# CaiLiLab/MuRaL

Measured on AMD Instinct MI355X. Metric: predicted bases/s (SNV local=10/distal=1000, 4-class, predict), higher is better.
Workload: dtype f32; 1 GPU; SNV default predict, synthetic 10M positions (BASELINE.json configs[1]); local_radius=10, distal_radius=1000, n_class=4, input=2-bit packed genome resident in HBM, every site's full window, weights=weights_init, torch.manual_seed(0), parallelism=dp1, collective=none

## Files before the change

include/mural_hip_debug.h:

```cpp
#ifndef MURAL_HIP_DEBUG_H
#define MURAL_HIP_DEBUG_H
#include "mural_hip.h"

#ifdef __cplusplus
extern "C" {
#endif

int mural_debug_last_ws_layout(size_t* out_pairs, int32_t max_pairs);

int mural_debug_run_scan(int64_t* v, int64_t m, int64_t stride, int32_t threads, int64_t* total, void* stream);

int mural_debug_cl_conv32_fwd(const float* x, int64_t B, int32_t L, int32_t pre_relu, const double* acc, const float* gamma,
                              const float* beta, float* running_mean, float* running_var, float* state, const float* W,
                              const float* bias, int32_t post_relu, const float* res1, const float* res2, double* acc_out,
                              int32_t out_relu, float* y, void* stream);
int mural_debug_cl_conv32_bwd(const float* dy, const float* x, const float* W, int64_t B, int32_t L, const float* state,
                              int32_t pre_relu, float* dz, double* stat_out, float* part, int32_t* nrow, void* stream);
int mural_debug_cl_bn_stats(const float* x, int64_t rows, int32_t relu, double* acc, void* stream);
int mural_debug_first_fwd_cl(const uint8_t* sym, int64_t B, int32_t Lwin, int32_t col0, int32_t L1, int32_t pk, int32_t ps, int32_t pp,
                             const float* gamma, const float* beta, const float* W, const float* bias, float eps, float momentum,
                             float* running_mean, float* running_var, unsigned long long* counts, float* tab, float* y, void* arg,
                             double* stat, void* stream);
int mural_debug_first_bwd_cl(const float* dy, const void* arg, const uint8_t* sym, int64_t B, int32_t Lwin, int32_t col0, int32_t L1,
                             int32_t pk, int32_t ps, int32_t pp, const float* tab, const float* W, float* scratch, float* dW,
// ... 28 lines not shown
                              int32_t out_relu, float* y, float* wfrag_scratch, void* stream);
int mural_debug_cw_conv32_bwd(const float* dy, const float* x, const float* W, int64_t B, int32_t L, const float* state,
                              const float* gamma, int32_t pre_relu, float* dz, double* stat_out, float* part, int32_t* nrow,
                              float* wfrag_scratch, void* stream);

int mural_debug_conv1d(const float* in, const float* wt, const float* bias, float* out, int64_t B, int32_t Cin, int32_t Lin,
                       int32_t Cout, int32_t Lout, int32_t K, int32_t stride, int32_t up, int32_t act, const float* res1,
                       const float* res2, int32_t engine, void* stream);

int mural_debug_poison_lds(void* stream);

int mural_debug_convblock(const float* x, const float* w5, const float* b5, const float* w1, const float* b1, const float* res2,
                          float* out, int64_t B, int32_t C, int32_t L, const float* f_in, const float* f_w, const float* f_b,
                          int32_t Cf, int32_t f_up, const float* f_pw, const float* ta_w, const float* ta_b, const float* tb_w,
                          const float* tb_b, float* tail_max, int32_t form, void* stream);

int mural_debug_conv1d_set_stamps(unsigned long long* stamps);
int mural_debug_cb8_set_stamps(unsigned long long* stamps);

int mural_debug_set_stamps(void* dev_ptr);

int mural_debug_list_switches(char* buf, size_t cap);

#ifdef __cplusplus
}
#endif
#endif
```

mural_amd/_lib.py:

```python
import ctypes as C
import os

import torch

_HERE = os.path.dirname(os.path.abspath(__file__))
LIB_PATH = os.path.join(_HERE, "libmural_hip.so")

MURAL_OK, MURAL_E_INVALID, MURAL_E_RUNTIME, MURAL_E_WORKSPACE, MURAL_E_ENCODING = 0, 1, 2, 3, 4

_f32p = C.POINTER(C.c_float)


class MuralGenome(C.Structure):
    _fields_ = [("packed2", C.c_void_p), ("nmask", C.c_void_p), ("length", C.c_int64), ("amb_pos", C.c_void_p),
                ("amb_sym", C.c_void_p), ("n_amb", C.c_int64)]


class MuralBN(C.Structure):
    _fields_ = [("weight", C.c_void_p), ("bias", C.c_void_p), ("running_mean", C.c_void_p), ("running_var", C.c_void_p)]


class MuralAffine(C.Structure):
    _fields_ = [("weight", C.c_void_p), ("bias", C.c_void_p)]

# ... 315 lines not shown
    "mural_debug_first_set_stamps": (C.c_int, [VP]),
    "mural_debug_lt_set_stamps": (C.c_int, [VP]),
    "mural_debug_cw_conv32_fwd": (C.c_int, [VP, I64, I32, I32, VP, VP, VP, VP, VP, VP, VP, VP, I32, VP, VP, VP, I32, VP, VP, VP]),
    "mural_debug_cw_conv32_bwd": (C.c_int, [VP, VP, VP, I64, I32, VP, VP, I32, VP, VP, VP, VP, VP, VP]),
    "mural_debug_cl_bn_stats": (C.c_int, [VP, I64, I32, VP, VP]),
    "mural_debug_local_train_fwd": (C.c_int, [VP, VP, I32, I32, I64, VP, VP, VP, VP, VP, VP, VP, VP, VP, VP, VP, VP, C.c_float, C.c_float, VP,
                                              VP, VP, VP]),
    "mural_debug_local_train_bwd": (C.c_int, [VP, I32, I32, I64, VP, VP, VP, VP, VP, VP, VP, VP, VP, VP, VP, VP, VP, VP, VP, VP, VP, VP, VP]),
    "mural_debug_head_train_fwd": (C.c_int, [VP, I64, I32, VP, VP, VP, VP, VP, C.c_float, C.c_float, VP, VP, VP, C.c_float, C.c_uint64, VP, VP,
                                             VP, VP, I32, VP, VP]),
    "mural_debug_head_train_bwd": (C.c_int, [VP, VP, I32, I64, I32, VP, VP, VP, C.c_float, C.c_uint64, VP, VP, VP, VP, VP, VP, VP, VP, VP, VP,
                                             VP, VP]),
    "mural_debug_first_fwd_cl": (C.c_int, [VP, I64, I32, I32, I32, I32, I32, I32, VP, VP, VP, VP, C.c_float, C.c_float, VP, VP, VP, VP, VP, VP,
                                           VP, VP]),
    "mural_debug_first_bwd_cl": (C.c_int, [VP, VP, VP, I64, I32, I32, I32, I32, I32, I32, VP, VP, VP, VP, VP, VP, VP, VP, VP, VP, VP, VP, VP,
                                           VP, C.c_double, VP, VP, VP]),
    "mural_debug_conv1d": (C.c_int, [VP, VP, VP, VP, I64, I32, I32, I32, I32, I32, I32, I32, I32, VP, VP, I32, VP]),
    "mural_debug_conv1d_set_stamps": (C.c_int, [VP]),
    "mural_debug_poison_lds": (C.c_int, [VP]),
    "mural_debug_convblock": (C.c_int, [VP, VP, VP, VP, VP, VP, VP, I64, I32, I32, VP, VP, VP, I32, I32, VP, VP, VP, VP, VP, VP, I32, VP]),
    "mural_debug_cb8_set_stamps": (C.c_int, [VP]),
    "mural_debug_set_stamps": (C.c_int, [C.c_void_p]),
    "mural_debug_list_switches": (C.c_int, [C.c_char_p, C.c_size_t]),
}

_lib = None
DEBUG_LIB_PATH = os.path.join(_HERE, "libmural_hip_debug.so")


def flavor():
    return "debug" if os.environ.get("MURAL_HIP_FLAVOR", "") == "debug" else "product"


def lib():
    global _lib
    if _lib is None:
        debug = flavor() == "debug"
        path = DEBUG_LIB_PATH if debug else LIB_PATH
        if not os.path.exists(path):
            raise RuntimeError(
                f"{path} is missing: the HIP extension has not been built. "
                "Run `make -C mural_amd/csrc` (needs hipcc, --offload-arch=gfx950). There is no CPU fallback.")
        handle = C.CDLL(path)
        protos = dict(PROTOTYPES, **DEBUG_PROTOTYPES) if debug else PROTOTYPES
        for name, (res, args) in protos.items():
            fn = getattr(handle, name)
# ... 25 lines not shown
```

mural_amd/csrc/debug_hooks.hip:

```cpp
#include <cstring>
#include <string>
#include <vector>

#include "../../include/mural_hip_debug.h"
#include "common.h"
#include "conv1d.h"
#include "conv32_cl.h"
#include "conv32_jobs.h"
#include "snv.h"
#include "train_ops.h"

using namespace mural;

#define STREAM ((hipStream_t)stream)

namespace {
struct EnableDevSwitches {
  EnableDevSwitches() { mural::g_dev_switches = true; }
} g_enable_dev_switches;
}

extern "C" int mural_debug_list_switches(char* buf, size_t cap) {
  std::string text;
  int n = 0;
  for (const mural::DevSwitch* s = mural::dev_switch_table(); s->name; ++s, ++n) text += std::string(s->name) + "\t" + s->what + "\n";
  if (buf && cap) {
    std::strncpy(buf, text.c_str(), cap - 1);
    buf[cap - 1] = '\0';
  }
  return n;
}

__global__ __launch_bounds__(256) void lds_poison_kernel(float* sink) {
  extern __shared__ float lds_all[];
  for (int i = threadIdx.x; i < 160 * 256; i += 256) lds_all[i] = __builtin_nanf("");
  __syncthreads();
  if (sink && lds_all[(threadIdx.x * 97) % (160 * 256)] == 1.f) sink[0] = 1.f;
}
static int poison_lds(hipStream_t stream) {
  MURAL_HIP_CHECK(hipFuncSetAttribute(reinterpret_cast<const void*>(lds_poison_kernel), hipFuncAttributeMaxDynamicSharedMemorySize, 160 * 1024));
  hipLaunchKernelGGL(lds_poison_kernel, dim3(2048), dim3(256), 160 * 1024, stream, (float*)nullptr);
  MURAL_HIP_CHECK(hipGetLastError());
  return MURAL_OK;
}

extern "C" int mural_debug_conv1d_set_stamps(unsigned long long* stamps) {
  mural::conv1d_mfma_set_stamps(stamps);
  return MURAL_OK;
}

extern "C" int mural_debug_cb8_set_stamps(unsigned long long* stamps) {
  mural::g_cb8_stamps = stamps;
  return MURAL_OK;
// ... 239 lines not shown
```

mural_amd/csrc/encode.hip:

```cpp
#include <cstring>
#include <cstdlib>
#include "common.h"
#include "dense_symbol.h"

namespace mural {

static thread_local std::string g_err;

void set_error(const char* fmt, ...) {
  char buf[1024];
  va_list ap;
  va_start(ap, fmt);
  vsnprintf(buf, sizeof(buf), fmt, ap);
  va_end(ap);
  g_err = buf;
}

const char* last_error_cstr() { return g_err.c_str(); }

bool g_dev_switches = false;

const DevSwitch* dev_switch_table() {
  static const DevSwitch table[] = {
    {"MURAL_TOWER_DYNAMIC_UNITS", "A/B, bit-identical: SNV predict units through a global ticket counter instead of the fixed stride"},
    {"MURAL_SNV_DEFER_SHORT", "A/B, bit-identical: =0 runs the short-stage launches per chunk (what a one-chunk workspace does by itself)"},
    {"MURAL_LOCAL_REG", "A/B, bit-identical: =0 keeps the local MLP's weight fragments in LDS (snv_local_mlp_mfma)"},
    {"MURAL_INDEL_CHUNK", "A/B, same results: positions per pass of the INDEL layer program (256 .. 4096; default 2048)"},
    {"MURAL_TRAIN_CONV_CL", "A/B: the training step on the workgroup-tile conv kernels (conv32_cl.hip) instead of the wave-private ones"},
    {"MURAL_TRAIN_NO_FIRST_FOLD", "A/B: the first stage's last BatchNorm-backward apply as a pass of its own"},
    {"MURAL_TRAIN_NO_MID_FOLD", "A/B: the short stage's last apply as a pass of its own"},
    {"MURAL_TRAIN_NO_POOL_FOLD", "A/B: the applies in front of the pools as passes of their own"},
    {"MURAL_TRAIN_LOCAL_OPS", "A/B: the local branch of the training step as per-op launches"},
    {"MURAL_TRAIN_HEAD_OPS", "A/B: a tower's head of the training step as per-op launches"},
    {"MURAL_TRAIN_FIRST_SEPARATE", "A/B: symbol histograms / first-layer tables per tower"},
    {"MURAL_XCD_SWIZZLE", "A/B, bit-identical: =0 disables the XCD-aware workgroup index of the barrier-free INDEL kernels"},
    {"MURAL_CONVBLOCK_DIRECT", "A/B: 0 / 2 never / always the barrier-free ConvBlock"},
    {"MURAL_CONVBLOCK8_VALU", "A/B: the 8-channel ConvBlock entirely on the vector ALU"},
    {"MURAL_INDEL_ENC0", "A/B: =0 disables the persistent level-0 encoder launch"},
    {"MURAL_INDEL_ENC0_DOWN", "A/B: =0 keeps the stride-4 down-conv a launch of its own"},
    {"MURAL_INDEL_DEC0", "A/B: =0 disables the persistent level-0 decoder launch"},
    {"MURAL_INDEL_DEEP", "A/B: =0 runs the deep levels' blocks as two launches each"},
    {"MURAL_INDEL_DEEP_FRONT", "A/B: =0 keeps the fourth level's strided conv a launch of its own"},
    {"MURAL_INDEL_DENSE_SYMBOLS", "A/B: =0 keeps the dense INDEL entry on the three-launch route"},
    {"MURAL_WGRAD_MFMA", "A/B: =0 keeps the INDEL weight gradients on the LDS-tiled vector kernel"},
    {"MURAL_DEBUG_WS_GUARD", "validation: unused bytes behind every workspace region (tests poison and check them)"},
    {"MURAL_DEBUG_DROP_PART_ROW", "validation (fault injection): drop one partial row of a conv weight gradient"},
    {"MURAL_DEBUG_NO_SMALL_BATCH", "validation: calls of <= 256 sites through the throughput launches"},
    {"MURAL_DEBUG_NO_LONGWIN", "validation: long windows through the per-layer path"},
// ... 240 lines not shown
```

mural_amd/csrc/snv.h:

```cpp
#pragma once
#include "common.h"

namespace mural {

constexpr int SNV_C = 32;
constexpr int SNV_K = 3;
constexpr int SNV_NLAYER = 10;
constexpr int SNV_KSTEPS = 24;
constexpr int SNV_WFRAG = 2 * SNV_KSTEPS * 64;
constexpr int SNV_LUT = 125 * SNV_C;
constexpr int SNV_TAPS = 3 * N_SYM * SNV_C;
constexpr int SNV_LUTBLK = SNV_LUT + SNV_TAPS + SNV_C;
constexpr int SNV_LUT4 = 256 * SNV_C;
constexpr int SNV_MAXCLASS = 16;
constexpr int SNV_CHUNK = 131072;
constexpr int SNV_NB2MAX = 9;
constexpr int SNV_THREADS = 256;
constexpr int SNV_WAVES = SNV_THREADS / 64;
constexpr int SNV_MID_HALF = 100;

enum { L_RB1A_C1 = 0, L_RB1A_C2, L_RB1B_C1, L_RB1B_C2, L_CONV2, L_RB2A_C1, L_RB2A_C2, L_RB2B_C1, L_RB2B_C2, L_CONV3 };
enum { EX_RB1_ENTRY = 0, EX_BN_MID = 1, EX_BN_OUT = 2, EX_FC_BN = 3, EX_COUNT = 4 };

struct TowerGeom {
// ... 172 lines not shown
  float* blob;
  size_t blob_floats;
  size_t lds_bytes;
  mural::Stage1Args s1;
  size_t s1_lds_bytes;
  bool s1_pair;
  bool loc_fused;
  mural::LocalMfmaDims loc_d;
  size_t loc_lds;
  bool longwin;
  bool front_only;
  bool front_mid;
  int lw_nA, lw_LA, lw_LB, lw_SB, lw_nj;
  mural::SnvFwdArgs args_lwA, args_lwB;
  size_t lds_lwA, lds_lwB;
  int64_t chunk;
};

namespace mural {
bool stage1_small_batch(int64_t n);
int launch_snv_stage1(const Stage1Args& a, bool packed, size_t lds_bytes, hipStream_t stream);
int launch_snv_local(const LocalDev& L, const int64_t* cat, int64_t n, float* out, hipStream_t stream);
int launch_snv_towers(const MuralSnvModel* m, const SnvFwdArgs& a, size_t lds_bytes, hipStream_t stream);
int profile_begin();
int profile_end(double* total_ms, int64_t* launches);
size_t plan_wave_geometry(SnvFwdArgs& a, int Lwin, int Pw, int n_class, int tower, int phase);
int launch_snv_tower_wave(const SnvFwdArgs& a, size_t lds_bytes, hipStream_t stream);
int launch_snv_tower_wave_jobs(const SnvFwdArgs* jobs, const size_t* lds_bytes, int n, hipStream_t stream);
extern unsigned long long* g_tower_stamps;
}
```

mural_amd/csrc/snv_model.hip:

```cpp
#include <algorithm>
#include <cmath>
#include <cstdio>
#include <cstdlib>
#include <cstring>
#include <vector>

#include "snv.h"
#include "snv_local_mfma.h"

namespace mural {

namespace {

const double kSymVec[15][4] = {
    {1, 0, 0, 0}, {0, 1, 0, 0}, {0, 0, 1, 0}, {0, 0, 0, 1}, {.25, .25, .25, .25},
    {.5, 0, .5, 0}, {0, .5, 0, .5}, {.5, .5, 0, 0}, {0, .5, .5, 0}, {.5, 0, 0, .5}, {0, 0, .5, .5},
    {0, 1. / 3, 1. / 3, 1. / 3}, {1. / 3, 0, 1. / 3, 1. / 3}, {1. / 3, 1. / 3, 0, 1. / 3}, {1. / 3, 1. / 3, 1. / 3, 0}};

struct Blob {
  std::vector<float> host;
  size_t alloc(size_t n) {
    size_t off = (host.size() + 63) & ~size_t(63);
    host.resize(off + n, 0.f);
    return off;
// ... 341 lines not shown
          if (need && need <= kLdsTwoPerCu) { Pq = cand; m->lds_split[q] = need; }
        }
        if (!Pq) return false;
        if (phase == 2) {
          for (int cand = Pq; cand >= Pq - 2 && cand >= 1; --cand) {
            SnvFwdArgs tmp;
            const size_t need = plan_geometry(tmp, sh.distal_len, cand, sh.n_class, towers, phase);
            if (need && tmp.geom[q & 1].nb[1] % 4 == 0) { Pq = cand; m->lds_split[q] = need; break; }
          }
        }
        plan_geometry(m->args_split[q], sh.distal_len, Pq, sh.n_class, towers, phase);
        for (int cand = 31; cand >= 1; --cand) {
          SnvFwdArgs tmp;
          std::memset(&tmp, 0, sizeof(tmp));
          const size_t need = plan_wave_geometry(tmp, sh.distal_len, cand, sh.n_class, q & 1, phase);
          if (need && need <= kLdsTwoPerCu) {
            m->args_split[q] = tmp;
            m->lds_split[q] = need;
            break;
          }
        }
        return true;
      };
      m->chunk = SNV_CHUNK;
      m->longwin = false;
      if (!dev_env("MURAL_DEBUG_NO_LONGWIN")) {
        SnvFwdArgs probe;
        std::memset(&probe, 0, sizeof(probe));
        fill_tower_lengths(probe, sh.distal_len);
        const int L2 = probe.geom[0].L[0], nj = 19, LA = 7 * nj + 8;
        if (L2 > LA && probe.geom[0].pk[1] == 7 && probe.geom[0].ps[1] == 7 && probe.geom[0].pp[1] == 3) {
          int nA = 0;
          while (7 * nj * nA + LA <= L2) ++nA;
          const int SB = 7 * ((L2 - 142 + 6) / 7), LB = L2 - SB;
          bool ok = nA >= 1 && LB >= 127 && LB <= 142 && SB <= 7 * nj * nA && SB >= 0;
          if (ok) {
            std::memset(&m->args_lwA, 0, sizeof(SnvFwdArgs));
            std::memset(&m->args_lwB, 0, sizeof(SnvFwdArgs));
            m->lds_lwA = plan_wave_geometry(m->args_lwA, 15 * (LA - 1) + 1, 1, sh.n_class, 0, 1);
            m->lds_lwB = plan_wave_geometry(m->args_lwB, 15 * (LB - 1) + 1, 1, sh.n_class, 0, 1);
            ok = m->lds_lwA && m->lds_lwA <= kLdsTwoPerCu && m->lds_lwB && m->lds_lwB <= kLdsTwoPerCu &&
                 m->args_lwA.geom[0].L[0] == LA && m->args_lwB.geom[0].L[0] == LB;
          }
          bool part_ok[4] = {ok, false, false, false};
          for (int q = 1; q < 4 && ok; ++q) part_ok[q] = plan_part(q);
          const bool short_ok = ok && part_ok[1] && part_ok[2] && part_ok[3];
          if (ok) {
// ... 127 lines not shown
extern "C" int mural_snv_tap_layout(const MuralSnvModel* m, int32_t* o) {
  MURAL_REQUIRE(m && o, "NULL argument");
  std::memset(o, 0, 16 * sizeof(int32_t));
  o[0] = m->args.P;
  o[1] = m->args.nbuf;
  for (int i = 0; i < 3; ++i) { o[2 + i] = m->args.geom[0].L[i]; o[5 + i] = m->args.geom[1].L[i]; }
  o[8] = 13;
  o[9] = (int32_t)m->lds_bytes;
  o[10] = m->front_only ? 1 : 0;
  o[11] = (int32_t)m->chunk;
  o[12] = m->front_mid ? 1 : 0;
  return MURAL_OK;
}

extern "C" const char* mural_snv_kernel_name(void) { return "snv_tower_wave"; }

extern "C" int mural_profile_begin(void) { return mural::profile_begin(); }
extern "C" int mural_profile_end(double* total_ms, int64_t* launches) { return mural::profile_end(total_ms, launches); }

namespace mural { unsigned long long* g_tower_stamps = nullptr; }

constexpr int64_t SNV_SMALL_BATCH = 256;

static int run_towers(const MuralSnvModel* m, Stage1Args s1, SnvFwdArgs a, bool packed, int64_t n, const Workspace& w,
                      float* out, float* taps, const int32_t* status, hipStream_t stream, bool one_chunk = false, float* front_out = nullptr) {
  const int nc = m->shape.n_class;
  const bool small = taps == nullptr && n <= SNV_SMALL_BATCH && m->lds_small > 0 && !dev_env("MURAL_DEBUG_NO_SMALL_BATCH");
  const bool defer = m->split && taps == nullptr && !small && !m->longwin && super_chunk_sites(m) > m->chunk && n > m->chunk && !one_chunk;
  const int64_t super = defer ? super_chunk_sites(m) : m->chunk;
  const size_t s3l_site = (size_t)std::max(m->args.geom[0].L[1], 1) * SNV_C, s3m_site = (size_t)std::max(m->args.geom[1].L[1], 1) * SNV_C;
  for (int64_t sc0 = 0; sc0 < n; sc0 += super) {
  const int64_t sn = std::min<int64_t>(super, n - sc0);
  for (int64_t c0 = sc0; c0 < sc0 + sn; c0 += m->chunk) {
    const int64_t cn = std::min<int64_t>(m->chunk, sc0 + sn - c0);
    const int64_t rel = defer ? c0 - sc0 : 0;
    Stage1Args s = s1;
    s.n = cn;
    s.x0 = w.x0;
    s.zero = small ? reinterpret_cast<int*>(w.s3[1]) : nullptr;
    if (packed) { s.pos = s1.pos + c0; s.strand = s1.strand + c0; }
    else s.codes = s1.codes + c0 * m->shape.distal_len;
    if (int rc = launch_snv_stage1(s, packed, s.loc_on ? std::max(m->s1_lds_bytes, m->loc_lds) : m->s1_lds_bytes, stream)) return rc;
    const bool split = m->split && taps == nullptr && !small;
    if (split && dev_int("MURAL_TOWER_DYNAMIC_UNITS", 0) != 0)
      MURAL_HIP_CHECK(hipMemsetAsync(w.counters, 0, 64, stream));
    bool lw_mid_done = false;
    for (int part = 0; part < (split ? (defer ? 2 : 4) : 1); ++part) {
      if (part == 1 && lw_mid_done) continue;
      if (m->longwin && part == 0) {
        const int LpA = m->args_lwA.geom[0].L[1], LpB = m->args_lwB.geom[0].L[1], L3 = m->args.geom[0].L[1], nj = m->lw_nj;
        const int x0_cols = m->args.x0_cols;
        auto grid_of = [](int64_t items) { return dim3((unsigned)std::min<int64_t>((items + 255) / 256, 65536)); };
        SnvFwdArgs lw_jobs[3];
        size_t lw_lds[3];
        const bool lw_merge = m->args_lwA.wave && m->args_lwB.wave && m->args_split[1].wave && (!front_out || m->front_mid);
        for (int kind = 0; kind < 2; ++kind) {
          SnvFwdArgs t = kind == 0 ? m->args_lwA : m->args_lwB;
          t.n = kind == 0 ? cn * m->lw_nA : cn;
          t.x0 = w.x0;
          t.x0_cols = x0_cols;
          t.seg_n = kind == 0 ? m->lw_nA : 1;
          t.seg_step = kind == 0 ? 7 * nj : 0;
          t.seg_col0 = kind == 0 ? 0 : m->lw_SB;
          t.s3[0] = kind == 0 ? w.vs3A : w.vs3B;
          t.s3[1] = w.s3[1];
          t.xlogit = w.xlogit;
          t.local_logits = w.local_logits + c0 * nc;
          t.out = out ? out + c0 * nc : nullptr;
          t.taps = nullptr;
          t.stamps = nullptr;
// ... 16 lines not shown
          t.local_logits = w.local_logits + c0 * nc;
          t.out = out ? out + c0 * nc : nullptr;
          t.taps = nullptr;
          t.tap_stride = a.nbuf;
          t.stamps = nullptr;
          t.status = status;
          t.unit_counter = nullptr;
          lw_jobs[2] = t;
          lw_lds[2] = m->lds_split[1];
          if (int rc = launch_snv_tower_wave_jobs(lw_jobs, lw_lds, 3, stream)) return rc;
          lw_mid_done = true;
        }
        const int jA = m->lw_nA * nj + 1;
        float* s3_dst = front_out ? front_out + (size_t)c0 * L3 * SNV_C : w.s3[0];
        hipLaunchKernelGGL(lw_scatter_kernel, grid_of(cn * jA * 8), dim3(256), 0, stream, w.vs3A, cn, m->lw_nA, LpA, nj, 0, jA, 0, L3, s3_dst);
        if (L3 > jA)
          hipLaunchKernelGGL(lw_scatter_kernel, grid_of(cn * (L3 - jA) * 8), dim3(256), 0, stream, w.vs3B, cn, 1, LpB, nj, jA, L3,
                             -(m->lw_SB / 7), L3, s3_dst);
        MURAL_HIP_CHECK(hipGetLastError());
        if (front_out && !m->front_mid) break;
        continue;
      }
      if (front_out && part > 1) break;
      SnvFwdArgs t = split ? m->args_split[part] : (small ? m->args_small : a);
      t.s3[0] = w.s3[0] + (size_t)rel * s3l_site;
      t.s3[1] = w.s3[1] + (size_t)rel * s3m_site;
      t.n = cn;
      t.x0 = w.x0;
      t.xlogit = w.xlogit + (size_t)rel * SNV_MAXCLASS;
      if (small) {
        t.par = 1;
        t.xlogit2 = w.s3[0];
        t.tile_count = reinterpret_cast<int*>(w.s3[1]);
      }
      t.local_logits = w.local_logits + c0 * nc;
      t.out = out ? out + c0 * nc : nullptr;
      t.taps = c0 == 0 ? taps : nullptr;
      t.tap_stride = a.nbuf;
      t.stamps = packed ? mural::g_tower_stamps : nullptr;
      t.status = status;
      t.unit_counter = split && t.wave ? w.counters + part : nullptr;
      size_t lds = split ? m->lds_split[part] : (small ? m->lds_small : m->lds_bytes);
      if (split && !t.wave && part >= 2 && t.P > 1) {
        const int want = (int)std::max<int64_t>(1, std::min<int64_t>(t.P, (cn + 511) / 512));
        if (want < t.P) {
          SnvFwdArgs t2 = t;
          const size_t need = plan_geometry(t2, m->shape.distal_len, want, m->shape.n_class, (part & 1) ? 2 : 1, 2);
          if (need && need <= lds) {
            t = t2;
            lds = need;
          }
        }
      }
      if (int rc = launch_snv_towers(m, t, lds, stream)) return rc;
    }
  }
  if (defer) {
    for (int part = 2; part < 4; ++part) {
      SnvFwdArgs t = m->args_split[part];
      t.s3[0] = w.s3[0];
      t.s3[1] = w.s3[1];
      t.n = sn;
      t.x0 = w.x0;
      t.xlogit = w.xlogit;
// ... 191 lines not shown
```

mural_amd/csrc/snv_tower.hip:

```cpp
#include <cstdlib>
#include <vector>

#include "snv_tower_conv.h"

namespace mural {

#define SNV_STAMP(id)                                                              \
  do {                                                                             \
    if (args.stamps != nullptr && tid == 0) {                                      \
      const unsigned long long _t = __builtin_amdgcn_s_memtime();                  \
      args.stamps[(size_t)blockIdx.x * 32 + (id)] += _t - t_prev;                  \
      t_prev = _t;                                                                 \
    }                                                                              \
  } while (0)

__device__ __forceinline__ void request_x0(const SnvFwdArgs& args, f32x4 (&xres)[SNV_NB2MAX], int64_t tile, int tw_i,
                                           int64_t n_tiles, int cgp, int n16, int chv) {
  const TowerGeom& g = args.geom[tw_i];
  const int x0c = tw_i == 0 ? 0 : args.geom[0].L[0];
  const int nbw0 = g.nb[0] > cgp ? (g.nb[0] - cgp + 1) / 2 : 0;
  const float* base = args.x0 + (size_t)x0c * 32 + chv;
#pragma unroll
  for (int i = 0; i < SNV_NB2MAX; ++i) {
    xres[i] = splat(0.f);
// ... 379 lines not shown
}

int profile_begin() {
  g_prof.on = true;
  g_prof.used = 0;
  return MURAL_OK;
}

int profile_end(double* total_ms, int64_t* launches) {
  double sum = 0.0;
  for (size_t i = 0; i + 1 < g_prof.used; i += 2) {
    MURAL_HIP_CHECK(hipEventSynchronize(g_prof.ev[i + 1]));
    float ms = 0.f;
    MURAL_HIP_CHECK(hipEventElapsedTime(&ms, g_prof.ev[i], g_prof.ev[i + 1]));
    sum += ms;
  }
  if (total_ms) *total_ms = sum;
  if (launches) *launches = (int64_t)(g_prof.used / 2);
  g_prof.on = false;
  g_prof.used = 0;
  return MURAL_OK;
}

int launch_snv_towers(const MuralSnvModel* m, const SnvFwdArgs& a, size_t lds_bytes, hipStream_t stream) {
  const int64_t n_tiles = (a.n + a.P - 1) / a.P;
  if (n_tiles == 0) return MURAL_OK;
  if (a.wave) {
    hipEvent_t w0 = nullptr, w1 = nullptr;
    if (g_prof.on) {
      while (g_prof.ev.size() < g_prof.used + 2) {
        hipEvent_t e;
        MURAL_HIP_CHECK(hipEventCreate(&e));
        g_prof.ev.push_back(e);
      }
      w0 = g_prof.ev[g_prof.used];
      w1 = g_prof.ev[g_prof.used + 1];
      g_prof.used += 2;
      MURAL_HIP_CHECK(hipEventRecord(w0, stream));
    }
    if (int rc = launch_snv_tower_wave(a, lds_bytes, stream)) return rc;
    if (w1) MURAL_HIP_CHECK(hipEventRecord(w1, stream));
    return MURAL_OK;
  }
  int grid = (int)(n_tiles < 2048 ? n_tiles : 2048);
  if (a.par) grid = (int)(2 * n_tiles);
  static DynLdsOnce big_lds;
  if (int rc = big_lds.ensure(&snv_towers_fused<0>, &snv_towers_fused<1>, &snv_towers_fused<2>, &snv_towers_fused<3>)) return rc;
  hipEvent_t e0 = nullptr, e1 = nullptr;
  if (g_prof.on) {
    while (g_prof.ev.size() < g_prof.used + 2) {
      hipEvent_t e;
      MURAL_HIP_CHECK(hipEventCreate(&e));
      g_prof.ev.push_back(e);
    }
    e0 = g_prof.ev[g_prof.used];
    e1 = g_prof.ev[g_prof.used + 1];
    g_prof.used += 2;
    MURAL_HIP_CHECK(hipEventRecord(e0, stream));
  }
  if (a.par) hipLaunchKernelGGL(snv_towers_fused<3>, dim3(grid), dim3(SNV_THREADS), lds_bytes, stream, a);
  else if (a.phase == 1) hipLaunchKernelGGL(snv_towers_fused<1>, dim3(grid), dim3(SNV_THREADS), lds_bytes, stream, a);
  else if (a.phase == 2) hipLaunchKernelGGL(snv_towers_fused<2>, dim3(grid), dim3(SNV_THREADS), lds_bytes, stream, a);
  else hipLaunchKernelGGL(snv_towers_fused<0>, dim3(grid), dim3(SNV_THREADS), lds_bytes, stream, a);
  MURAL_HIP_CHECK(hipGetLastError());
  if (e1) MURAL_HIP_CHECK(hipEventRecord(e1, stream));
  return MURAL_OK;
}

}
```

mural_amd/csrc/snv_tower_wave.hip:

```cpp
#include <cstdlib>
#include <cstring>
#include <type_traits>

#include "snv_tower_conv.h"

namespace mural {

template <int M>
using ModeTag = std::integral_constant<int, M>;
__host__ __device__ constexpr TowerGeom wave_tower_geom(int tw, int Lwin, int Pw) {
  constexpr int pools[2][3][3] = {{{15, 15, 7}, {7, 7, 3}, {3, 3, 1}}, {{3, 3, 1}, {3, 3, 1}, {3, 3, 1}}};
  TowerGeom g{};
  g.L1 = tw == 0 ? Lwin : 2 * SNV_MID_HALF + 1;
  g.col0 = tw == 0 ? 0 : Lwin / 2 - SNV_MID_HALF;
  int L = g.L1;
  for (int i = 0; i < 3; ++i) {
    g.pk[i] = pools[tw][i][0];
    g.ps[i] = pools[tw][i][1];
    g.pp[i] = pools[tw][i][2];
    L = (L + 2 * g.pp[i] - g.pk[i]) / g.ps[i] + 1;
    g.L[i] = L;
    if (L < 1) return g;
    g.Sc[i] = L + 1;
    g.NC[i] = 1 + Pw * g.Sc[i];
    g.nb[i] = (g.NC[i] + 15) / 16;
    g.dL[i] = FastDiv::make((uint32_t)L);
    g.dSc[i] = FastDiv::make((uint32_t)g.Sc[i]);
  }
  return g;
}
constexpr int SHIP_LWIN = 2001;

constexpr int MODE_GENERIC = -1;
constexpr int TW_NBW = 9;
constexpr int TW_DUMP = 128;
constexpr uint32_t TW_BLK = 2048u;

struct WaveAddr {
  uint32_t rd[6];
  uint32_t wr[2];
  uint32_t vmask;
  uint32_t dump;
};

__device__ __forceinline__ WaveAddr wave_setup(const TowerGeom& g, int st, int Pw, int n16, int kk, uint32_t dump0) {
  WaveAddr a;
  a.dump = dump0 + 16u * (uint32_t)((16 * kk + n16) & 31);
#pragma unroll
// ... 262 lines not shown
template <int PHASE, int NBA, int NBB, int TWC = -1, int PWC = 0>
__global__ __launch_bounds__(SNV_THREADS, 2) void snv_tower_wave(const SnvFwdArgs args) {
#define SNVW_BX blockIdx.x
#define SNVW_GX gridDim.x
#include "snv_tower_wave_body.inc"
}
#undef SNVW_BX
#undef SNVW_GX

struct SnvFwdJobs {
  SnvFwdArgs j[3];
  int grid[3];
};
static_assert(sizeof(SnvFwdJobs) <= 4096, "kernel arguments: 4 KB");
#define SNVW_BX bx_job
#define SNVW_GX gx_job
template <int PHASE, int NBA, int NBB, int TWC = -1, int PWC = 0>
__global__ __launch_bounds__(SNV_THREADS, 2) void snv_tower_wave_jobs(const SnvFwdJobs jobs) {
  const SnvFwdArgs& args = jobs.j[blockIdx.y];
  const unsigned gx_job = (unsigned)jobs.grid[blockIdx.y];
  const unsigned bx_job = blockIdx.x;
  if (bx_job >= gx_job) return;
#include "snv_tower_wave_body.inc"
}
#undef SNVW_BX
#undef SNVW_GX

constexpr int EW_NB = 9;
constexpr int EW_WST = 32;

__device__ __forceinline__ int64_t edge_wave_wstart(const EdgeArgs& args, int64_t row) {
  if (row >= args.n) return -1;
  const int64_t gp = args.pos[row];
  const int neg = args.strand[row] != 0;
  const int64_t t = neg ? args.glen - 1 - gp : gp;
  const int64_t w = t + args.woff - args.t0[neg];
  if (w < 0 || w + args.L1 > args.nb || args.F[neg] == nullptr) return -1;
  return w | ((int64_t)neg << 62);
}

__device__ __forceinline__ void edge_wave_request(const EdgeArgs& args, const int64_t* wst, f32x4 (&xr0)[TW_NBW], f32x4 (&xr1)[TW_NBW],
                                                  int n16_in, int kk) {
  int n16 = n16_in;
  asm volatile("" : "+v"(n16));
  const float* safe = args.F[0] != nullptr ? args.F[0] : args.F[1];
#pragma unroll
// ... 214 lines not shown
static bool tower_dynamic_units() { return dev_int("MURAL_TOWER_DYNAMIC_UNITS", 0) != 0; }

size_t edge_wave_lds_bytes() {
  return (size_t)(4 * SNV_C + 4 * 3 * SNV_C + SNV_WAVES * ((16 * EW_NB + 2) * SNV_C + EW_WST + TW_DUMP)) * 4;
}

int launch_snv_edge_wave(const EdgeArgs& e, int* unit_counter, hipStream_t stream) {
  const int64_t n_units = (e.n + EW_P - 1) / EW_P;
  const int64_t n_wg = (n_units + SNV_WAVES - 1) / SNV_WAVES;
  if (n_wg == 0) return MURAL_OK;
  const int grid = (int)(n_wg < 512 ? n_wg : 512);
  if (n_units < 4 * (int64_t)grid * SNV_WAVES || !tower_dynamic_units()) unit_counter = nullptr;
  static DynLdsOnce lds;
  if (int rc = lds.ensure(&snv_edge_wave)) return rc;
  hipLaunchKernelGGL(snv_edge_wave, dim3(grid), dim3(SNV_THREADS), edge_wave_lds_bytes(), stream, e, unit_counter);
  MURAL_HIP_CHECK(hipGetLastError());
  return MURAL_OK;
}

size_t plan_wave_geometry(SnvFwdArgs& a, int Lwin, int Pw, int n_class, int tower, int phase) {
  int maxcols = 0;
  for (int tw = 0; tw < 2; ++tw) {
    a.geom[tw] = wave_tower_geom(tw, Lwin, Pw);
    const TowerGeom& g = a.geom[tw];
    for (int i = 0; i < 3; ++i) {
      if (g.L[i] < 1) return 0;
      if (tw != tower) continue;
      if ((phase == 1 && i != 0) || (phase == 2 && i == 0)) continue;
      if (g.nb[i] > TW_NBW) return 0;
      if (phase == 1 && g.nb[i] != TW_NBW) return 0;
      maxcols = std::max(maxcols, 16 * g.nb[i] + 2);
    }
  }
  if (Pw > 31) return 0;
  if (phase == 2 && !(Lwin == SHIP_LWIN && Pw == (tower == 0 ? 6 : 5))) return 0;
  a.P = Pw;
  a.Lwin = Lwin;
  a.tw_first = tower;
  a.tw_last = tower;
  a.phase = phase;
  a.wave = 1;
  a.x0_cols = a.geom[0].L[0] + a.geom[1].L[0];
  a.nbuf = maxcols * SNV_C;
  const size_t par = (size_t)(2 * EX_COUNT * SNV_C + n_class * SNV_C + SNV_MAXCLASS + 4 + 6 * 3 * SNV_C);
  const size_t per_wave = (size_t)a.nbuf + (phase == 2 ? (size_t)Pw * SNV_C + 3 * (size_t)Pw * SNV_MAXCLASS : 0) + TW_DUMP;
  return (par + SNV_WAVES * per_wave) * 4;
// ... 10 lines not shown
    const SnvFwdArgs& a = jobs_in[i];
    MURAL_REQUIRE(a.phase == 1 && a.Lwin != SHIP_LWIN, "wave-private tower jobs: first-stage launches of the run-time-geometry instance only");
    const int64_t n_units = (a.n + a.P - 1) / a.P;
    const int64_t n_wg = (n_units + SNV_WAVES - 1) / SNV_WAVES;
    if (n_wg == 0) continue;
    jobs.j[ny] = a;
    jobs.j[ny].unit_counter = nullptr;
    wg_of[ny] = n_wg;
    lds = lds_bytes[i] > lds ? lds_bytes[i] : lds;
    ++ny;
  }
  if (ny == 0) return MURAL_OK;
  for (int i = 0; i < ny; ++i) {
    jobs.grid[i] = (int)(wg_of[i] < 512 ? wg_of[i] : 512);
    gx = jobs.grid[i] > gx ? jobs.grid[i] : gx;
  }
  static DynLdsOnce big_lds;
  if (int rc = big_lds.ensure(&snv_tower_wave_jobs<1, 9, 0>)) return rc;
  hipLaunchKernelGGL((snv_tower_wave_jobs<1, 9, 0>), dim3(gx, ny), dim3(SNV_THREADS), lds, stream, jobs);
  MURAL_HIP_CHECK(hipGetLastError());
  return MURAL_OK;
}

int launch_snv_tower_wave(const SnvFwdArgs& a_in, size_t lds_bytes, hipStream_t stream) {
  SnvFwdArgs a = a_in;
  const int64_t n_units = (a.n + a.P - 1) / a.P;
  const int64_t n_wg = (n_units + SNV_WAVES - 1) / SNV_WAVES;
  if (n_wg == 0) return MURAL_OK;
  const int resident = 512;
  const int grid = (int)(n_wg < resident ? n_wg : resident);
  if (n_units < 4 * (int64_t)grid * SNV_WAVES || !tower_dynamic_units()) a.unit_counter = nullptr;
  static DynLdsOnce big_lds;
  if (int rc = big_lds.ensure(&snv_tower_wave<1, 9, 0, 0, 1>, &snv_tower_wave<1, 9, 0, 1, 2>, &snv_tower_wave<2, 8, 4, 0, 6>,
                              &snv_tower_wave<2, 8, 3, 1, 5>, &snv_tower_wave<1, 9, 0>)) return rc;
  const int t = a.tw_first;
  const int ship_pw = a.phase == 1 ? (t == 0 ? 1 : 2) : (t == 0 ? 6 : 5);
  bool ship = a.Lwin == SHIP_LWIN && a.P == ship_pw && !(a.phase == 1 && dev_env("MURAL_DEBUG_TOWER_RUNTIME_GEOM"));
  if (ship) {
    const TowerGeom want = wave_tower_geom(t, SHIP_LWIN, ship_pw), other = wave_tower_geom(0, SHIP_LWIN, 1);
    const TowerGeom& have = a.geom[t];
    for (int i = 0; i < 3; ++i)
      ship = ship && have.L[i] == want.L[i] && have.Sc[i] == want.Sc[i] && have.NC[i] == want.NC[i] && have.nb[i] == want.nb[i] &&
             have.pk[i] == want.pk[i] && have.ps[i] == want.ps[i] && have.pp[i] == want.pp[i];
    ship = ship && a.geom[0].L[0] == other.L[0] && a.x0_cols == other.L[0] + wave_tower_geom(1, SHIP_LWIN, 1).L[0];
  }
  const dim3 gr(grid), bl(SNV_THREADS);
  if (a.phase == 1) {
    if (ship && t == 0) hipLaunchKernelGGL((snv_tower_wave<1, 9, 0, 0, 1>), gr, bl, lds_bytes, stream, a);
    else if (ship) hipLaunchKernelGGL((snv_tower_wave<1, 9, 0, 1, 2>), gr, bl, lds_bytes, stream, a);
    else hipLaunchKernelGGL((snv_tower_wave<1, 9, 0>), gr, bl, lds_bytes, stream, a);
  } else {
    if (ship && t == 0) hipLaunchKernelGGL((snv_tower_wave<2, 8, 4, 0, 6>), gr, bl, lds_bytes, stream, a);
    else if (ship) hipLaunchKernelGGL((snv_tower_wave<2, 8, 3, 1, 5>), gr, bl, lds_bytes, stream, a);
    else {
      set_error("internal: short-stage wave launch without the shipped geometry");
      return MURAL_E_INVALID;
    }
  }
  MURAL_HIP_CHECK(hipGetLastError());
  return MURAL_OK;
}

}
```

mural_amd/csrc/snv_tower_wave_body.inc:

```
  extern __shared__ __attribute__((aligned(16))) float smem[];
  const int tid = threadIdx.x;
  const int lane = tid & 63;
  const int wave = __builtin_amdgcn_readfirstlane(tid >> 6);
  const int n16 = lane & 15, kk = lane >> 4;
  constexpr bool SHIP = TWC >= 0;
  const int Pw = SHIP ? PWC : args.P;
  const int tw_i = SHIP ? TWC : args.tw_first;
  unsigned long long t_prev = args.stamps != nullptr ? __builtin_amdgcn_s_memtime() : 0ull;
  if (args.stamps != nullptr && lane == 0) {
    unsigned long long* row = args.stamps + (size_t)(1024 + 2 * SNVW_BX + (wave >> 1)) * 32;
    row[((PHASE - 1) * 2 + tw_i) * 4 + 2 * (wave & 1)] = __builtin_amdgcn_s_memrealtime();
    if (PHASE == 1 && tw_i == 0) {
      row[16 + 2 * (wave & 1)] = __builtin_amdgcn_s_getreg((31 << 11) | (0 << 6) | 4);
      row[17 + 2 * (wave & 1)] = __builtin_amdgcn_s_getreg((3 << 11) | (0 << 6) | 20);
    }
  }
  constexpr TowerGeom g_ship = wave_tower_geom(SHIP ? TWC : 0, SHIP_LWIN, SHIP ? PWC : 1);
  const TowerGeom& g_arg = args.geom[SHIP ? 0 : tw_i];
  const TowerGeom& g = SHIP ? g_ship : g_arg;
  const TowerDev& tw = args.tw[tw_i];
  const int L0_large = SHIP ? wave_tower_geom(0, SHIP_LWIN, 1).L[0] : args.geom[0].L[0];
  const int x0_cols = SHIP ? wave_tower_geom(0, SHIP_LWIN, 1).L[0] + wave_tower_geom(1, SHIP_LWIN, 1).L[0] : args.x0_cols;
  const int x0c = tw_i == 0 ? 0 : L0_large;
  const int lpar0 = 2 * EX_COUNT * SNV_C + args.n_class * SNV_C + SNV_MAXCLASS + 4;
  const int par_floats = lpar0 + 6 * 3 * SNV_C;
  float* par = smem;
  const int wave_floats = args.nbuf + (PHASE == 2 ? Pw * SNV_C + 3 * Pw * SNV_MAXCLASS : 0) + TW_DUMP;
  const uint32_t dump0 = 4u * (uint32_t)(wave_floats - TW_DUMP);
  float* img = smem + par_floats + wave * wave_floats;
  float* feat = img + args.nbuf;
  float* logit = feat + Pw * SNV_C;
  for (int i = tid; i < EX_COUNT * SNV_C; i += SNV_THREADS) {
    par[i] = tw.ex_s[i];
    par[EX_COUNT * SNV_C + i] = tw.ex_t[i];
  }
  for (int i = tid; i < args.n_class * SNV_C; i += SNV_THREADS) par[2 * EX_COUNT * SNV_C + i] = tw.fc_w[i];
  if (tid < args.n_class) par[2 * EX_COUNT * SNV_C + args.n_class * SNV_C + tid] = tw.fc_b[tid];
  {
    const int l0 = PHASE == 1 ? 0 : 4, nl = PHASE == 1 ? 4 : 6;
    for (int i = tid; i < nl * SNV_C; i += SNV_THREADS) {
// ... 318 lines not shown
```

Before: 17.20 million bases/s.

## Merge first-stage large/mid tower launches into one paired kernel and quantize chunks

Adds a paired kernel that runs the large and mid first-stage towers of a chunk in one launch using a 2D grid (blockIdx.y selects the tower). This removes a launch and the gap between the two, letting both towers' workgroups share the GPU. Chunk lengths are now cut to a multiple of a quantum derived from the two towers' sites per unit, so every chunk fills whole units. The block count per tower geometry now drops the extra padding column, which shrinks one phase-2 instance's NBA/NBB from 4 to 3. The paired launch sizes LDS for the larger tower, which may reduce occupancy for the smaller one.

```diff
diff --git a/include/mural_hip_debug.h b/include/mural_hip_debug.h
--- a/include/mural_hip_debug.h
+++ b/include/mural_hip_debug.h
@@ -74,6 +74,9 @@
 
 int mural_debug_list_switches(char* buf, size_t cap);
 
+int mural_debug_snv_chunk_cut(int64_t n, int64_t cap, int64_t quantum, int64_t* out, int32_t max);
+int64_t mural_debug_wave_geometry(int32_t lwin, int32_t pw, int32_t n_class, int32_t tower, int32_t phase, int32_t* out);
+
 #ifdef __cplusplus
 }
 #endif
diff --git a/mural_amd/_lib.py b/mural_amd/_lib.py
--- a/mural_amd/_lib.py
+++ b/mural_amd/_lib.py
@@ -361,6 +361,8 @@
     "mural_debug_cb8_set_stamps": (C.c_int, [VP]),
     "mural_debug_set_stamps": (C.c_int, [C.c_void_p]),
     "mural_debug_list_switches": (C.c_int, [C.c_char_p, C.c_size_t]),
+    "mural_debug_snv_chunk_cut": (C.c_int, [I64, I64, I64, VP, I32]),
+    "mural_debug_wave_geometry": (C.c_int64, [I32, I32, I32, I32, I32, VP]),
 }
 
 _lib = None
diff --git a/mural_amd/csrc/debug_hooks.hip b/mural_amd/csrc/debug_hooks.hip
--- a/mural_amd/csrc/debug_hooks.hip
+++ b/mural_amd/csrc/debug_hooks.hip
@@ -29,6 +29,33 @@
     buf[cap - 1] = '\0';
   }
   return n;
+}
+
+extern "C" int mural_debug_snv_chunk_cut(int64_t n, int64_t cap, int64_t quantum, int64_t* out, int32_t max) {
+  if (n < 0 || cap < 1 || quantum < 1 || (!out && max > 0)) return -2;
+  int k = 0;
+  for (int64_t left = n; left > 0; ++k) {
+    const int64_t cn = mural::snv_chunk_len(left, cap, quantum);
+    if (k >= max) return -1;
+    out[k] = cn;
+    left -= cn;
+  }
+  return k;
+}
+
+extern "C" int64_t mural_debug_wave_geometry(int32_t lwin, int32_t pw, int32_t n_class, int32_t tower, int32_t phase, int32_t* out) {
+  if (!out || tower < 0 || tower > 1 || pw < 1 || lwin < 1) return 0;
+  mural::SnvFwdArgs a;
+  std::memset(&a, 0, sizeof(a));
+  const size_t lds = mural::plan_wave_geometry(a, lwin, pw, n_class, tower, phase);
+  const mural::TowerGeom& g = a.geom[tower];
+  for (int i = 0; i < 3; ++i) {
+    out[i] = g.L[i];
+    out[3 + i] = g.Sc[i];
+    out[6 + i] = g.NC[i];
+    out[9 + i] = g.nb[i];
+  }
+  return (int64_t)lds;
 }
 
 __global__ __launch_bounds__(256) void lds_poison_kernel(float* sink) {
diff --git a/mural_amd/csrc/encode.hip b/mural_amd/csrc/encode.hip
--- a/mural_amd/csrc/encode.hip
+++ b/mural_amd/csrc/encode.hip
@@ -24,6 +24,8 @@
   static const DevSwitch table[] = {
     {"MURAL_TOWER_DYNAMIC_UNITS", "A/B, bit-identical: SNV predict units through a global ticket counter instead of the fixed stride"},
     {"MURAL_SNV_DEFER_SHORT", "A/B, bit-identical: =0 runs the short-stage launches per chunk (what a one-chunk workspace does by itself)"},
+    {"MURAL_SNV_LAUNCH_PLAN", "A/B, bit-identical: =0 runs the two first-stage tower launches of a chunk separately and cuts chunks at the plain cap"},
+    {"MURAL_SNV_CHUNK", "A/B, bit-identical: sites per stage-1 / tower launch sequence of a model created while it is set (256 .. 131072)"},
     {"MURAL_LOCAL_REG", "A/B, bit-identical: =0 keeps the local MLP's weight fragments in LDS (snv_local_mlp_mfma)"},
     {"MURAL_INDEL_CHUNK", "A/B, same results: positions per pass of the INDEL layer program (256 .. 4096; default 2048)"},
     {"MURAL_TRAIN_CONV_CL", "A/B: the training step on the workgroup-tile conv kernels (conv32_cl.hip) instead of the wave-private ones"},
diff --git a/mural_amd/csrc/snv.h b/mural_amd/csrc/snv.h
--- a/mural_amd/csrc/snv.h
+++ b/mural_amd/csrc/snv.h
@@ -218,10 +218,14 @@
 int launch_snv_stage1(const Stage1Args& a, bool packed, size_t lds_bytes, hipStream_t stream);
 int launch_snv_local(const LocalDev& L, const int64_t* cat, int64_t n, float* out, hipStream_t stream);
 int launch_snv_towers(const MuralSnvModel* m, const SnvFwdArgs& a, size_t lds_bytes, hipStream_t stream);
+int launch_snv_tower_pair(const SnvFwdArgs& large, size_t lds_large, const SnvFwdArgs& mid, size_t lds_mid, hipStream_t stream);
 int profile_begin();
 int profile_end(double* total_ms, int64_t* launches);
 size_t plan_wave_geometry(SnvFwdArgs& a, int Lwin, int Pw, int n_class, int tower, int phase);
 int launch_snv_tower_wave(const SnvFwdArgs& a, size_t lds_bytes, hipStream_t stream);
 int launch_snv_tower_wave_jobs(const SnvFwdArgs* jobs, const size_t* lds_bytes, int n, hipStream_t stream);
+bool snv_tower_wave_pairs(const SnvFwdArgs& large, const SnvFwdArgs& mid);
+int launch_snv_tower_wave_pair(const SnvFwdArgs& large, size_t lds_large, const SnvFwdArgs& mid, size_t lds_mid, hipStream_t stream);
+int64_t snv_chunk_len(int64_t left, int64_t cap, int64_t quantum);
 extern unsigned long long* g_tower_stamps;
 }
diff --git a/mural_amd/csrc/snv_model.hip b/mural_amd/csrc/snv_model.hip
--- a/mural_amd/csrc/snv_model.hip
+++ b/mural_amd/csrc/snv_model.hip
@@ -387,7 +387,7 @@
         }
         return true;
       };
-      m->chunk = SNV_CHUNK;
+      m->chunk = std::min(std::max(dev_int("MURAL_SNV_CHUNK", SNV_CHUNK), 256), SNV_CHUNK);
       m->longwin = false;
       if (!dev_env("MURAL_DEBUG_NO_LONGWIN")) {
         SnvFwdArgs probe;
@@ -561,6 +561,21 @@
 
 constexpr int64_t SNV_SMALL_BATCH = 256;
 
+static bool merged_launch_plan() { return dev_int("MURAL_SNV_LAUNCH_PLAN", 1) != 0; }
+
+int64_t mural::snv_chunk_len(int64_t left, int64_t cap, int64_t quantum) {
+  if (left <= cap) return left;
+  return cap >= quantum && quantum > 0 ? cap / quantum * quantum : cap;
+}
+static int64_t chunk_quantum(const MuralSnvModel* m) {
+  if (!m->split || !merged_launch_plan()) return 1;
+  const SnvFwdArgs &l = m->longwin ? m->args_lwB : m->args_split[0], &d = m->args_split[1];
+  if (!l.wave || !d.wave) return 1;
+  int a = l.P, b = d.P;
+  while (b) { const int r = a % b; a = b; b = r; }
+  return (int64_t)512 * SNV_WAVES * (l.P / a * d.P);
+}
+
 static int run_towers(const MuralSnvModel* m, Stage1Args s1, SnvFwdArgs a, bool packed, int64_t n, const Workspace& w,
                       float* out, float* taps, const int32_t* status, hipStream_t stream, bool one_chunk = false, float* front_out = nullptr) {
   const int nc = m->shape.n_class;
@@ -570,8 +585,9 @@
   const size_t s3l_site = (size_t)std::max(m->args.geom[0].L[1], 1) * SNV_C, s3m_site = (size_t)std::max(m->args.geom[1].L[1], 1) * SNV_C;
   for (int64_t sc0 = 0; sc0 < n; sc0 += super) {
   const int64_t sn = std::min<int64_t>(super, n - sc0);
-  for (int64_t c0 = sc0; c0 < sc0 + sn; c0 += m->chunk) {
-    const int64_t cn = std::min<int64_t>(m->chunk, sc0 + sn - c0);
+  const int64_t quantum = chunk_quantum(m);
+  for (int64_t c0 = sc0, cn = 0; c0 < sc0 + sn; c0 += cn) {
+    cn = snv_chunk_len(sc0 + sn - c0, m->chunk, quantum);
     const int64_t rel = defer ? c0 - sc0 : 0;
     Stage1Args s = s1;
     s.n = cn;
@@ -583,8 +599,37 @@
     const bool split = m->split && taps == nullptr && !small;
     if (split && dev_int("MURAL_TOWER_DYNAMIC_UNITS", 0) != 0)
       MURAL_HIP_CHECK(hipMemsetAsync(w.counters, 0, 64, stream));
+    auto part_args = [&](int part) {
+      SnvFwdArgs t = split ? m->args_split[part] : (small ? m->args_small : a);
+      t.s3[0] = w.s3[0] + (size_t)rel * s3l_site;
+      t.s3[1] = w.s3[1] + (size_t)rel * s3m_site;
+      t.n = cn;
+      t.x0 = w.x0;
+      t.xlogit = w.xlogit + (size_t)rel * SNV_MAXCLASS;
+      if (small) {
+        t.par = 1;
+        t.xlogit2 = w.s3[0];
+        t.tile_count = reinterpret_cast<int*>(w.s3[1]);
+      }
+      t.local_logits = w.local_logits + c0 * nc;
+      t.out = out ? out + c0 * nc : nullptr;
+      t.taps = c0 == 0 ? taps : nullptr;
+      t.tap_stride = a.nbuf;
+      t.stamps = packed ? mural::g_tower_stamps : nullptr;
+      t.status = status;
+      t.unit_counter = split && t.wave ? w.counters + part : nullptr;
+      return t;
+    };
     bool lw_mid_done = false;
-    for (int part = 0; part < (split ? (defer ? 2 : 4) : 1); ++part) {
+    int part0 = 0;
+    if (split && !m->longwin && !front_out && merged_launch_plan()) {
+      const SnvFwdArgs tl = part_args(0), tm = part_args(1);
+      if (snv_tower_wave_pairs(tl, tm)) {
+        if (int rc = launch_snv_tower_pair(tl, m->lds_split[0], tm, m->lds_split[1], stream)) return rc;
+        part0 = 2;
+      }
+    }
+    for (int part = part0; part < (split ? (defer ? 2 : 4) : 1); ++part) {
       if (part == 1 && lw_mid_done) continue;
       if (m->longwin && part == 0) {
         const int LpA = m->args_lwA.geom[0].L[1], LpB = m->args_lwB.geom[0].L[1], L3 = m->args.geom[0].L[1], nj = m->lw_nj;
@@ -647,24 +692,7 @@
         continue;
       }
       if (front_out && part > 1) break;
-      SnvFwdArgs t = split ? m->args_split[part] : (small ? m->args_small : a);
-      t.s3[0] = w.s3[0] + (size_t)rel * s3l_site;
-      t.s3[1] = w.s3[1] + (size_t)rel * s3m_site;
-      t.n = cn;
-      t.x0 = w.x0;
-      t.xlogit = w.xlogit + (size_t)rel * SNV_MAXCLASS;
-      if (small) {
-        t.par = 1;
-        t.xlogit2 = w.s3[0];
-        t.tile_count = reinterpret_cast<int*>(w.s3[1]);
-      }
-      t.local_logits = w.local_logits + c0 * nc;
-      t.out = out ? out + c0 * nc : nullptr;
-      t.taps = c0 == 0 ? taps : nullptr;
-      t.tap_stride = a.nbuf;
-      t.stamps = packed ? mural::g_tower_stamps : nullptr;
-      t.status = status;
-      t.unit_counter = split && t.wave ? w.counters + part : nullptr;
+      SnvFwdArgs t = part_args(part);
       size_t lds = split ? m->lds_split[part] : (small ? m->lds_small : m->lds_bytes);
       if (split && !t.wave && part >= 2 && t.P > 1) {
         const int want = (int)std::max<int64_t>(1, std::min<int64_t>(t.P, (cn + 511) / 512));
diff --git a/mural_amd/csrc/snv_tower.hip b/mural_amd/csrc/snv_tower.hip
--- a/mural_amd/csrc/snv_tower.hip
+++ b/mural_amd/csrc/snv_tower.hip
@@ -425,22 +425,35 @@
   return MURAL_OK;
 }
 
+static int profile_launch(hipStream_t stream, hipEvent_t* e0, hipEvent_t* e1) {
+  *e0 = *e1 = nullptr;
+  if (!g_prof.on) return MURAL_OK;
+  while (g_prof.ev.size() < g_prof.used + 2) {
+    hipEvent_t e;
+    MURAL_HIP_CHECK(hipEventCreate(&e));
+    g_prof.ev.push_back(e);
+  }
+  *e0 = g_prof.ev[g_prof.used];
+  *e1 = g_prof.ev[g_prof.used + 1];
+  g_prof.used += 2;
+  MURAL_HIP_CHECK(hipEventRecord(*e0, stream));
+  return MURAL_OK;
+}
+
+int launch_snv_tower_pair(const SnvFwdArgs& large, size_t lds_large, const SnvFwdArgs& mid, size_t lds_mid, hipStream_t stream) {
+  hipEvent_t w0, w1;
+  if (int rc = profile_launch(stream, &w0, &w1)) return rc;
+  if (int rc = launch_snv_tower_wave_pair(large, lds_large, mid, lds_mid, stream)) return rc;
+  if (w1) MURAL_HIP_CHECK(hipEventRecord(w1, stream));
+  return MURAL_OK;
+}
+
 int launch_snv_towers(const MuralSnvModel* m, const SnvFwdArgs& a, size_t lds_bytes, hipStream_t stream) {
   const int64_t n_tiles = (a.n + a.P - 1) / a.P;
   if (n_tiles == 0) return MURAL_OK;
   if (a.wave) {
-    hipEvent_t w0 = nullptr, w1 = nullptr;
-    if (g_prof.on) {
-      while (g_prof.ev.size() < g_prof.used + 2) {
-        hipEvent_t e;
-        MURAL_HIP_CHECK(hipEventCreate(&e));
-        g_prof.ev.push_back(e);
-      }
-      w0 = g_prof.ev[g_prof.used];
-      w1 = g_prof.ev[g_prof.used + 1];
-      g_prof.used += 2;
-      MURAL_HIP_CHECK(hipEventRecord(w0, stream));
-    }
+    hipEvent_t w0, w1;
+    if (int rc = profile_launch(stream, &w0, &w1)) return rc;
     if (int rc = launch_snv_tower_wave(a, lds_bytes, stream)) return rc;
     if (w1) MURAL_HIP_CHECK(hipEventRecord(w1, stream));
     return MURAL_OK;
@@ -449,18 +462,8 @@
   if (a.par) grid = (int)(2 * n_tiles);
   static DynLdsOnce big_lds;
   if (int rc = big_lds.ensure(&snv_towers_fused<0>, &snv_towers_fused<1>, &snv_towers_fused<2>, &snv_towers_fused<3>)) return rc;
-  hipEvent_t e0 = nullptr, e1 = nullptr;
-  if (g_prof.on) {
-    while (g_prof.ev.size() < g_prof.used + 2) {
-      hipEvent_t e;
-      MURAL_HIP_CHECK(hipEventCreate(&e));
-      g_prof.ev.push_back(e);
-    }
-    e0 = g_prof.ev[g_prof.used];
-    e1 = g_prof.ev[g_prof.used + 1];
-    g_prof.used += 2;
-    MURAL_HIP_CHECK(hipEventRecord(e0, stream));
-  }
+  hipEvent_t e0, e1;
+  if (int rc = profile_launch(stream, &e0, &e1)) return rc;
   if (a.par) hipLaunchKernelGGL(snv_towers_fused<3>, dim3(grid), dim3(SNV_THREADS), lds_bytes, stream, a);
   else if (a.phase == 1) hipLaunchKernelGGL(snv_towers_fused<1>, dim3(grid), dim3(SNV_THREADS), lds_bytes, stream, a);
   else if (a.phase == 2) hipLaunchKernelGGL(snv_towers_fused<2>, dim3(grid), dim3(SNV_THREADS), lds_bytes, stream, a);
diff --git a/mural_amd/csrc/snv_tower_wave.hip b/mural_amd/csrc/snv_tower_wave.hip
--- a/mural_amd/csrc/snv_tower_wave.hip
+++ b/mural_amd/csrc/snv_tower_wave.hip
@@ -23,7 +23,7 @@
     if (L < 1) return g;
     g.Sc[i] = L + 1;
     g.NC[i] = 1 + Pw * g.Sc[i];
-    g.nb[i] = (g.NC[i] + 15) / 16;
+    g.nb[i] = (Pw * g.Sc[i] + 15) / 16;
     g.dL[i] = FastDiv::make((uint32_t)L);
     g.dSc[i] = FastDiv::make((uint32_t)g.Sc[i]);
   }
@@ -332,6 +332,18 @@
   const unsigned bx_job = blockIdx.x;
   if (bx_job >= gx_job) return;
 #include "snv_tower_wave_body.inc"
+}
+
+template <int PHASE, int NBA, int NBB, int TWC, int PWC>
+__device__ __forceinline__ void snv_tower_wave_job(const SnvFwdArgs& args, const unsigned bx_job, const unsigned gx_job) {
+#include "snv_tower_wave_body.inc"
+}
+__global__ __launch_bounds__(SNV_THREADS, 2) void snv_tower_wave_pair(const SnvFwdJobs jobs) {
+  if (blockIdx.y == 0) {
+    if (blockIdx.x < (unsigned)jobs.grid[0]) snv_tower_wave_job<1, 9, 0, 0, 1>(jobs.j[0], blockIdx.x, (unsigned)jobs.grid[0]);
+  } else {
+    if (blockIdx.x < (unsigned)jobs.grid[1]) snv_tower_wave_job<1, 9, 0, 1, 2>(jobs.j[1], blockIdx.x, (unsigned)jobs.grid[1]);
+  }
 }
 #undef SNVW_BX
 #undef SNVW_GX
@@ -592,6 +604,7 @@
   int maxcols = 0;
   for (int tw = 0; tw < 2; ++tw) {
     a.geom[tw] = wave_tower_geom(tw, Lwin, Pw);
+    if (phase == 1 && tw == tower && a.geom[tw].L[0] >= 1 && Pw * a.geom[tw].Sc[0] == 16 * (TW_NBW - 1)) a.geom[tw].nb[0] = TW_NBW;
     const TowerGeom& g = a.geom[tw];
     for (int i = 0; i < 3; ++i) {
       if (g.L[i] < 1) return 0;
@@ -648,17 +661,7 @@
   return MURAL_OK;
 }
 
-int launch_snv_tower_wave(const SnvFwdArgs& a_in, size_t lds_bytes, hipStream_t stream) {
-  SnvFwdArgs a = a_in;
-  const int64_t n_units = (a.n + a.P - 1) / a.P;
-  const int64_t n_wg = (n_units + SNV_WAVES - 1) / SNV_WAVES;
-  if (n_wg == 0) return MURAL_OK;
-  const int resident = 512;
-  const int grid = (int)(n_wg < resident ? n_wg : resident);
-  if (n_units < 4 * (int64_t)grid * SNV_WAVES || !tower_dynamic_units()) a.unit_counter = nullptr;
-  static DynLdsOnce big_lds;
-  if (int rc = big_lds.ensure(&snv_tower_wave<1, 9, 0, 0, 1>, &snv_tower_wave<1, 9, 0, 1, 2>, &snv_tower_wave<2, 8, 4, 0, 6>,
-                              &snv_tower_wave<2, 8, 3, 1, 5>, &snv_tower_wave<1, 9, 0>)) return rc;
+static bool ship_geometry(const SnvFwdArgs& a) {
   const int t = a.tw_first;
   const int ship_pw = a.phase == 1 ? (t == 0 ? 1 : 2) : (t == 0 ? 6 : 5);
   bool ship = a.Lwin == SHIP_LWIN && a.P == ship_pw && !(a.phase == 1 && dev_env("MURAL_DEBUG_TOWER_RUNTIME_GEOM"));
@@ -670,13 +673,55 @@
              have.pk[i] == want.pk[i] && have.ps[i] == want.ps[i] && have.pp[i] == want.pp[i];
     ship = ship && a.geom[0].L[0] == other.L[0] && a.x0_cols == other.L[0] + wave_tower_geom(1, SHIP_LWIN, 1).L[0];
   }
+  return ship;
+}
+
+bool snv_tower_wave_pairs(const SnvFwdArgs& large, const SnvFwdArgs& mid) {
+  return large.wave && mid.wave && large.phase == 1 && mid.phase == 1 && large.tw_first == 0 && mid.tw_first == 1 && large.n > 0 &&
+         mid.n > 0 && large.seg_n == 0 && mid.seg_n == 0 && !tower_dynamic_units() && ship_geometry(large) && ship_geometry(mid);
+}
+
+int launch_snv_tower_wave_pair(const SnvFwdArgs& large, size_t lds_large, const SnvFwdArgs& mid, size_t lds_mid, hipStream_t stream) {
+  MURAL_REQUIRE(snv_tower_wave_pairs(large, mid), "internal: first-stage tower pair outside the shipped geometry");
+  SnvFwdJobs jobs;
+  std::memset(&jobs, 0, sizeof(jobs));
+  jobs.j[0] = large;
+  jobs.j[1] = mid;
+  int gx = 0;
+  for (int i = 0; i < 2; ++i) {
+    jobs.j[i].unit_counter = nullptr;
+    const int64_t n_units = (jobs.j[i].n + jobs.j[i].P - 1) / jobs.j[i].P;
+    const int64_t n_wg = (n_units + SNV_WAVES - 1) / SNV_WAVES;
+    jobs.grid[i] = (int)(n_wg < 512 ? n_wg : 512);
+    gx = jobs.grid[i] > gx ? jobs.grid[i] : gx;
+  }
+  static DynLdsOnce big_lds;
+  if (int rc = big_lds.ensure(&snv_tower_wave_pair)) return rc;
+  hipLaunchKernelGGL(snv_tower_wave_pair, dim3(gx, 2), dim3(SNV_THREADS), lds_large > lds_mid ? lds_large : lds_mid, stream, jobs);
+  MURAL_HIP_CHECK(hipGetLastError());
+  return MURAL_OK;
+}
+
+int launch_snv_tower_wave(const SnvFwdArgs& a_in, size_t lds_bytes, hipStream_t stream) {
+  SnvFwdArgs a = a_in;
+  const int64_t n_units = (a.n + a.P - 1) / a.P;
+  const int64_t n_wg = (n_units + SNV_WAVES - 1) / SNV_WAVES;
+  if (n_wg == 0) return MURAL_OK;
+  const int resident = 512;
+  const int grid = (int)(n_wg < resident ? n_wg : resident);
+  if (n_units < 4 * (int64_t)grid * SNV_WAVES || !tower_dynamic_units()) a.unit_counter = nullptr;
+  static DynLdsOnce big_lds;
+  if (int rc = big_lds.ensure(&snv_tower_wave<1, 9, 0, 0, 1>, &snv_tower_wave<1, 9, 0, 1, 2>, &snv_tower_wave<2, 8, 3, 0, 6>,
+                              &snv_tower_wave<2, 8, 3, 1, 5>, &snv_tower_wave<1, 9, 0>)) return rc;
+  const int t = a.tw_first;
+  const bool ship = ship_geometry(a);
   const dim3 gr(grid), bl(SNV_THREADS);
   if (a.phase == 1) {
     if (ship && t == 0) hipLaunchKernelGGL((snv_tower_wave<1, 9, 0, 0, 1>), gr, bl, lds_bytes, stream, a);
     else if (ship) hipLaunchKernelGGL((snv_tower_wave<1, 9, 0, 1, 2>), gr, bl, lds_bytes, stream, a);
     else hipLaunchKernelGGL((snv_tower_wave<1, 9, 0>), gr, bl, lds_bytes, stream, a);
   } else {
-    if (ship && t == 0) hipLaunchKernelGGL((snv_tower_wave<2, 8, 4, 0, 6>), gr, bl, lds_bytes, stream, a);
+    if (ship && t == 0) hipLaunchKernelGGL((snv_tower_wave<2, 8, 3, 0, 6>), gr, bl, lds_bytes, stream, a);
     else if (ship) hipLaunchKernelGGL((snv_tower_wave<2, 8, 3, 1, 5>), gr, bl, lds_bytes, stream, a);
     else {
       set_error("internal: short-stage wave launch without the shipped geometry");
diff --git a/mural_amd/csrc/snv_tower_wave_body.inc b/mural_amd/csrc/snv_tower_wave_body.inc
--- a/mural_amd/csrc/snv_tower_wave_body.inc
+++ b/mural_amd/csrc/snv_tower_wave_body.inc
@@ -16,6 +16,8 @@
     }
   }
   constexpr TowerGeom g_ship = wave_tower_geom(SHIP ? TWC : 0, SHIP_LWIN, SHIP ? PWC : 1);
+  static_assert(!SHIP || (PHASE == 1 ? NBA == g_ship.nb[0] : NBA == g_ship.nb[1] && NBB == g_ship.nb[2]),
+                "block counts of a compile-time-geometry instance are the geometry's");
   const TowerGeom& g_arg = args.geom[SHIP ? 0 : tw_i];
   const TowerGeom& g = SHIP ? g_ship : g_arg;
   const TowerDev& tw = args.tw[tw_i];
```

After: 17.37 million bases/s (median of 6 runs). Within noise of the previous version (+1.0%).
